# TheaQG/DiffusionModelsCustom

Hardware: NVIDIA B200
Metric: samples_per_s_T1000_ddpm_sampling (higher is better)
Workload: dtype fp16 operands, fp32 accumulate (fp32 state/update)

## Files before the change

### diffusionmodelscustom_b200/csrc/attention_tc8.cuh

```cuda
#pragma once
#include "attention_tc6.cuh"

namespace b2d {

constexpr int AT8_THREADS = 160;
constexpr int AT8_EQ_BYTES = ATC_BLK * ATC_D * 2;
constexpr int AT8_EK_BYTES = (ATC_BN / 2) * ATC_D * 2;
constexpr int AT8_SMEM = 1024 + ATC_TILE_BYTES + ATC_KV_BYTES * 3 * ATC_STAGES + AT8_EQ_BYTES + AT8_EK_BYTES + 256;

constexpr float AT8_OFF_SFU = 7.0f, AT8_OFF_POLY = 22.0f;

__device__ __forceinline__ uint32_t ex2_pair_poly_off(float xa, float xb) {
    uint32_t h, xr, nf, f, p, r;
    asm("cvt.rn.relu.f16x2.f32 %0, %1, %2;" : "=r"(h) : "f"(xb), "f"(xa));
    asm("add.rn.f16x2 %0, %1, %2;" : "=r"(xr) : "r"(h), "r"(0x66006600u));
    asm("sub.rn.f16x2 %0, %1, %2;" : "=r"(nf) : "r"(xr), "r"(0x66006600u));
    asm("sub.rn.f16x2 %0, %1, %2;" : "=r"(f) : "r"(h), "r"(nf));
    asm("fma.rn.f16x2 %0, %1, %2, %3;" : "=r"(p) : "r"(0x2B0D2B0Du), "r"(f), "r"(0x33C333C3u));
    asm("fma.rn.f16x2 %0, %1, %2, %3;" : "=r"(p) : "r"(p), "r"(f), "r"(0x398C398Cu));
    asm("fma.rn.f16x2 %0, %1, %2, %3;" : "=r"(p) : "r"(p), "r"(f), "r"(0x3C003C00u));
    const uint32_t e = xr * 1024u - 0x01980000u;
    asm("mul.rn.f16x2 %0, %1, %2;" : "=r"(r) : "r"(p), "r"(e));
    return r;
}

template <int POLY>
__global__ void __launch_bounds__(AT8_THREADS, AT6_CTAS_PER_SM)
    attn_tc8_kernel(const __grid_constant__ CUtensorMap tm, const __grid_constant__ CUtensorMap tmkv, f16* __restrict__ o, int L,
                    int C, float scale_log2e) {
    pdl_launch_dependents();
    extern __shared__ uint8_t at8_raw[];
    uint8_t* smem = reinterpret_cast<uint8_t*>((reinterpret_cast<uintptr_t>(at8_raw) + 1023) & ~uintptr_t(1023));
    uint8_t* sQ = smem;
    uint8_t* sK = sQ + ATC_TILE_BYTES;
    uint8_t* sV = sK + ATC_STAGES * ATC_KV_BYTES;
    uint8_t* sEq = sV + ATC_STAGES * 2 * ATC_KV_BYTES;
    uint8_t* sEk = sEq + AT8_EQ_BYTES;
    uint64_t* bars = reinterpret_cast<uint64_t*>(sEk + AT8_EK_BYTES);
    constexpr int KV_FULL = 0, S_FULL = 4 , P_EMPTY = 6, Q_FULL = 7, NBARS = 8;
    uint32_t* tmem_slot = reinterpret_cast<uint32_t*>(bars + NBARS);
    const uint32_t bar0 = smem_u32(bars);

    const int warp = threadIdx.x >> 5, lane = threadIdx.x & 31;
    const int head = blockIdx.y, b = blockIdx.z;
    const int q0 = blockIdx.x * ATC_BLK;
    const int nb = L / ATC_BN;
    const int row_base = b * L;
    constexpr int IW = 4, NT = AT8_THREADS;

    if (warp == IW) {
        if (lane == 0) {
            tma_prefetch_desc(&tm);
            tma_prefetch_desc(&tmkv);
            for (int i = 0; i < NBARS; ++i) mbar_init(&bars[i], 1);
            fence_mbar_init();
        }
        __syncwarp();
        tmem_alloc(tmem_slot, AT3_TMEM_COLS);
        tmem_relinquish();
    }
    for (int i = threadIdx.x; i < ATC_STAGES * ATC_BN * 2; i += NT) {
        const int st = i / (ATC_BN * 2), r = i % (ATC_BN * 2);
        *reinterpret_cast<uint4*>(sV + st * 2 * ATC_KV_BYTES + ATC_KV_BYTES + r * 16) = make_uint4(0x00003C00u, 0u, 0u, 0u);
    }
    for (int i = threadIdx.x; i < AT8_EQ_BYTES / 16; i += NT) *reinterpret_cast<uint4*>(sEq + i * 16) = make_uint4(0u, 0x00003C00u, 0u, 0u);
    for (int i = threadIdx.x; i < AT8_EK_BYTES / 16; i += NT) {
        const int pair = (i >> 1) >> 1;
        const uint32_t half_off = ((pair & 7) < POLY) ? 0x4980u  : 0x4300u ;
        *reinterpret_cast<uint4*>(sEk + i * 16) = make_uint4(0x38003800u, half_off, 0u, 0u);
    }
    fence_proxy_async();
    tc_fence_before();
    __syncthreads();
    tc_fence_after();
    const uint32_t tmem = *tmem_slot;
    pdl_wait();

    if (warp == IW) {
        constexpr uint32_t idesc_s = umma_idesc_f16_ex(128, ATC_BN / 2, 0);
        constexpr uint32_t idesc_o = umma_idesc_f16_ex(128, 2 * ATC_D, 1);
        const uint64_t dq = umma_desc(smem_u32(sQ), 0, 256, 6);
        const uint64_t dk0 = umma_desc(smem_u32(sK), 0, 256, 6);
        const uint64_t dv0 = umma_desc(smem_u32(sV), ATC_KV_BYTES, 256, 6);
        const uint64_t deq = umma_desc(smem_u32(sEq), 0, 256, 6);
        const uint64_t dek = umma_desc(smem_u32(sEk), 0, 256, 6);
        constexpr uint64_t K_HALF = (ATC_BN / 2) * ATC_D * 2 / 16;
        auto load_kv = [&](int t) {
            const int st = t & (ATC_STAGES - 1);
            mbar_arrive_expect_tx(&bars[KV_FULL + st], 2 * ATC_KV_BYTES);
            tma_load_2d(sK + st * ATC_KV_BYTES, &tmkv, &bars[KV_FULL + st], C + head * ATC_D, row_base + t * ATC_BN);
            tma_load_2d(sV + st * 2 * ATC_KV_BYTES, &tmkv, &bars[KV_FULL + st], 2 * C + head * ATC_D, row_base + t * ATC_BN);
        };
        auto issue_s_half = [&](int t, int ch) {
            const int ks = t & (ATC_STAGES - 1);
            mbar_wait_a(bar0 + 8 * (KV_FULL + ks), (t >> 2) & 1);
            tc_fence_after();
            const uint32_t d = tmem + ch * (ATC_BN / 2);
            umma_f16(d, dq, dk0 + (uint64_t)(ks * (ATC_KV_BYTES / 16)) + (uint64_t)ch * K_HALF, idesc_s, 0);
            umma_f16(d, deq, dek, idesc_s, 1);
            umma_commit_a(bar0 + 8 * (S_FULL + ch));
        };
        if (elect_one()) {
            mbar_arrive_expect_tx(&bars[Q_FULL], ATC_TILE_BYTES);
            tma_load_2d(sQ, &tm, &bars[Q_FULL], head * ATC_D, row_base + q0);
            const int pre = nb < ATC_STAGES ? nb : ATC_STAGES;
            for (int t = 0; t < pre; ++t) load_kv(t);
        }
// ... 103 lines not shown
                    }
                    if (__any_sync(0xffffffffu, move)) {
                        if (!waited_p) {
                            mbar_wait_a(bar0 + 8 * P_EMPTY, (j & 1) ^ 1);
                            tc_fence_after();
                            waited_p = true;
                        }
                        const float fac = move ? ex2_approx(m_ref - m_new) : 1.0f;
                        if (j > 0) rescale_o(fac);
                        if (ch == 1) rescale_p_first_half(fac);
                        if (j + 1 < nb) mbar_wait_a(bar0 + 8 * (S_FULL + 0), (j + 1) & 1);
                        if (ch == 0) mbar_wait_a(bar0 + 8 * (S_FULL + 1), j & 1);
                        else if (j + 1 < nb) mbar_wait_a(bar0 + 8 * (S_FULL + 1), (j + 1) & 1);
                        if (move) {
                            const f16 hi = __float2half_rn(m_new);
                            const f16 lo = __float2half_rn(m_new - __half2float(hi));
                            const uint32_t w = (uint32_t)__half_as_ushort(__hneg(hi)) | ((uint32_t)__half_as_ushort(__hneg(lo)) << 16);
                            eq_row[0] = w;
                            eq_row[4] = w;
                            m_eq = m_new;
                        }
                        fence_proxy_async();
                    }
                    const float shift = m_new - (m_ref - d0);
#pragma unroll
                    for (int i = 0; i < 32; ++i) v[i] = __float_as_uint(__uint_as_float(v[i]) - shift);
                    m_ref = m_new;
                }
                uint32_t pk[16];
#pragma unroll
                for (int idx = 0; idx < 16 + AT_PIPE; ++idx) {
                    if (idx < 16) {
                        const float s0 = __uint_as_float(v[2 * idx]), s1 = __uint_as_float(v[2 * idx + 1]);
                        if ((idx & 7) < POLY) {
                            pk[idx] = ex2_pair_poly_off(s0, s1);
                        } else {
                            v[2 * idx] = __float_as_uint(ex2_ordered(s0));
                            v[2 * idx + 1] = __float_as_uint(ex2_ordered(s1));
                        }
                    }
                    if (idx >= AT_PIPE) {
                        const int i = idx - AT_PIPE;
                        if ((i & 7) >= POLY) pk[i] = pack_h2_ordered(__uint_as_float(v[2 * i]), __uint_as_float(v[2 * i + 1]));
                    }
                }
                if (!waited_p) {
                    mbar_wait_a(bar0 + 8 * P_EMPTY, (j & 1) ^ 1);
                    tc_fence_after();
                    waited_p = true;
                }
                tmem_st16(tl + AT3_P_COL + ch * 16, pk);
            }
            tmem_st_wait();
            tc_fence_before();
            named_bar_arrive(3, NT);
        }
        mbar_wait_a(bar0 + 8 * P_EMPTY, (nb - 1) & 1);
        tc_fence_after();
        uint32_t ov[32];
        tmem_ld32(tl + AT3_O_COL, ov);
        tmem_ld_wait();
        const float inv = 1.0f / __uint_as_float(ov[16]);
        f16* op = o + ((size_t)(row_base + q0 + row)) * C + head * ATC_D;
        uint4 o0, o1;
        o0.x = pack_h2(__uint_as_float(ov[0]) * inv, __uint_as_float(ov[1]) * inv);
        o0.y = pack_h2(__uint_as_float(ov[2]) * inv, __uint_as_float(ov[3]) * inv);
        o0.z = pack_h2(__uint_as_float(ov[4]) * inv, __uint_as_float(ov[5]) * inv);
        o0.w = pack_h2(__uint_as_float(ov[6]) * inv, __uint_as_float(ov[7]) * inv);
        o1.x = pack_h2(__uint_as_float(ov[8]) * inv, __uint_as_float(ov[9]) * inv);
        o1.y = pack_h2(__uint_as_float(ov[10]) * inv, __uint_as_float(ov[11]) * inv);
        o1.z = pack_h2(__uint_as_float(ov[12]) * inv, __uint_as_float(ov[13]) * inv);
        o1.w = pack_h2(__uint_as_float(ov[14]) * inv, __uint_as_float(ov[15]) * inv);
        reinterpret_cast<uint4*>(op)[0] = o0;
        reinterpret_cast<uint4*>(op)[1] = o1;
    }
    tc_fence_before();
    __syncthreads();
    if (warp == IW) {
        tc_fence_after();
        tmem_dealloc(tmem, AT3_TMEM_COLS);
    }
}

inline int attn_tc8_poly() {
    static const int v = [] {
        const char* e = getenv("B2D_ATTN_POLY");
        const int p = e ? atoi(e) : 4;
        return p < 0 ? 0 : (p > 5 ? 5 : p);
    }();
    return v;
}

template <int POLY>
inline int attn_tc8_attr() {
    B2D_CUDA(cudaFuncSetAttribute(attn_tc8_kernel<POLY>, cudaFuncAttributeMaxDynamicSharedMemorySize, AT8_SMEM));
    B2D_CUDA(cudaFuncSetAttribute(attn_tc8_kernel<POLY>, cudaFuncAttributePreferredSharedMemoryCarveout, cudaSharedmemCarveoutMaxShared));
    return 0;
}
inline int attn_tc8_init_attrs() {
    B2D_TRY(attn_tc8_attr<0>());
    B2D_TRY(attn_tc8_attr<2>());
    B2D_TRY(attn_tc8_attr<3>());
    B2D_TRY(attn_tc8_attr<4>());
    B2D_TRY(attn_tc8_attr<5>());
    return 0;
}

inline int attn_tc8_launch(const AttnTcMaps& m, f16* o, int B, int L, int C, int heads, cudaStream_t st) {
    const float scale_log2e = 1.4426950408889634f / sqrtf((float)ATC_D);
    const dim3 grid(L / ATC_BLK, heads, B), block(AT8_THREADS);
    switch (attn_tc8_poly()) {
        case 0: case 1: B2D_CUDA(launch_k(attn_tc8_kernel<0>, grid, block, AT8_SMEM, st, m.q, m.kv, o, L, C, scale_log2e)); break;
        case 2: B2D_CUDA(launch_k(attn_tc8_kernel<2>, grid, block, AT8_SMEM, st, m.q, m.kv, o, L, C, scale_log2e)); break;
        case 3: B2D_CUDA(launch_k(attn_tc8_kernel<3>, grid, block, AT8_SMEM, st, m.q, m.kv, o, L, C, scale_log2e)); break;
        case 4: B2D_CUDA(launch_k(attn_tc8_kernel<4>, grid, block, AT8_SMEM, st, m.q, m.kv, o, L, C, scale_log2e)); break;
        default: B2D_CUDA(launch_k(attn_tc8_kernel<5>, grid, block, AT8_SMEM, st, m.q, m.kv, o, L, C, scale_log2e)); break;
    }
    return 0;
}

}
```

### diffusionmodelscustom_b200/csrc/b200ddpm.cu

```cuda
#include "../../include/b200ddpm.h"

#include <chrono>
#include <cmath>
#include <cstring>
#include <functional>
#include <map>
#include <memory>
#include <vector>

#include "attention.cuh"
#include "attention_tc.cuh"
#include "attention_tc2.cuh"
#include "attention_tc3.cuh"
#include "attention_tc3d32.cuh"
#include "attention_tc6.cuh"
#include "attention_tc8.cuh"
#include "attn_block.cuh"
#include "common.cuh"
#include "conv.cuh"
#include "conv_persist.cuh"
#include "elementwise.cuh"
#include "evalops.cuh"
#include "gemm_stream.cuh"
#include "norm_fused.cuh"
#include "tail_tc.cuh"

namespace b2d {
thread_local Status g_status;
int g_pdl_enabled = getenv("B2D_NO_PDL") ? 0 : 1;

static inline cudaStream_t as_stream(void* s) { return reinterpret_cast<cudaStream_t>(s); }

struct HostTensor {
    std::vector<float> v;
    std::vector<int64_t> shape;
    size_t numel() const { return v.size(); }
};

static inline uint16_t f2h(float f) {
    const float c = f > 65504.0f ? 65504.0f : (f < -65504.0f ? -65504.0f : f);
    const __half h = __float2half_rn(c);
    uint16_t u;
    memcpy(&u, &h, 2);
    return u;
}

typedef std::function<int(cudaStream_t)> OpFn;
struct Op {
    std::string name;
    std::string klass;
    double flops = 0;
    double bytes = 0;
    OpFn fn;
    bool side = false;
    bool join = false;
    int operator()(cudaStream_t st) const { return fn(st); }
};
struct OpList {
    std::vector<Op> v;
    Op pending;
    void meta(const std::string& name, const std::string& klass, double flops, double bytes) {
        pending.name = name; pending.klass = klass; pending.flops = flops; pending.bytes = bytes;
    }
    void push_back(OpFn f) {
        pending.fn = std::move(f);
        v.push_back(pending);
        pending = Op();
    }
};

struct EnsembleRes;
void ensemble_release(EnsembleRes* r);
struct Handle {
    b2d_config cfg{};
    int num_sms = 148;
    std::vector<void*> allocs;
    std::vector<void*> prog_allocs;
    bool in_prog = false;
    std::map<std::string, HostTensor> sd;
    std::map<std::string, void*> dev;
    bool weights_loaded = false;

    int T = 0;
    float *d_betas = nullptr, *d_alphas = nullptr, *d_alpha_hat = nullptr;

    int prog_B = 0;
    std::vector<Op> step_ops;
    size_t stats_floats = 0;
    float* d_stats = nullptr;
    const float* cur_x = nullptr;
    float* cur_eps = nullptr;
    float* d_eps = nullptr;
    int *d_t = nullptr, *d_step = nullptr, *d_y = nullptr;
    bool has_y = false, has_cond_set = false;
    float* d_cond_stack = nullptr;
    float* d_cond_pre = nullptr;
    float* d_temb = nullptr;
    int n_temb = 0;
    float* d_noise_stage = nullptr;
// ... 363 lines not shown
            auto gp = std::make_shared<GemmStreamPlan>();
            gp->p = p;
            if (gemm_stream_plan_build(*gp, h->num_sms) != 0) { err = -1; return; }
            ops.pending.klass = "gemm_stream";
            ops.push_back([gp](cudaStream_t st) { return gemm_stream_launch(*gp, st); });
        } else {
            if (conv_plan_build(*pl, h->num_sms) != 0) { err = -1; return; }
            static const bool no_gn_epi = getenv("B2D_NO_GN_EPILOGUE") != nullptr;
            const int hw_out = pl->p.Ho * pl->p.Wo;
            const bool gn_whole = pl->p.TN == 1;
            const bool gn_quarter = pl->p.TN > 1 && hw_out % 32 == 0;
            if (want_gn && !no_gn_epi && pl->p.splits == 1 && (gn_whole || gn_quarter) && !convt) {
                const int sub = gn_whole ? 1 : 4;
                const int mtiles = (int)pl->grid.x * sub, ntiles = (int)pl->grid.y;
                float* part = nullptr;
                if (h->alloc(&part, (size_t)mtiles * ntiles * 2) != 0) { err = -2; return; }
                pl->p.gn_partial = part;
                pl->p.gn_sub = sub;
                last_gn_partial = part;
                last_gn_tps = gn_whole ? pl->p.tiles_w * pl->p.tiles_h : hw_out / 32;
                last_gn_ntiles = ntiles;
                last_gn_mtiles = mtiles;
            }
            if (pl->ws_floats) {
                if (h->alloc(&pl->p.ws, pl->ws_floats) != 0) { err = -2; return; }
            }
            if (conv_tcp_eligible(*pl, h->num_sms)) {
                const int sms = h->num_sms;
                ops.pending.klass = "conv_tc";
                ops.push_back([pl, sms](cudaStream_t st) { return conv_launch_tcp(*pl, sms, st); });
            } else {
                ops.push_back([pl](cudaStream_t st) { return conv_launch_tc(*pl, st); });
            }
        }
    }

    f16 *s_xn = nullptr, *s_qkv = nullptr, *s_ao = nullptr, *s_h1 = nullptr, *s_mid = nullptr;

    void attention(const f16* x, int hw, int C, const std::string& role, f16* out, int final_act) {
        const int rows = B * hw * hw, L = hw * hw, heads = h->cfg.n_heads;
        const float* g = W<float>(role + ".ln.g");
        const float* b = W<float>(role + ".ln.b");
        f16 *xn = s_xn, *qkv = s_qkv, *ao = s_ao;
        const int Bc = B;
        static const bool no_ln_fold = getenv("B2D_NO_LN_FOLD") != nullptr;
        const bool fold = !no_ln_fold && !h->cfg.debug_simt_conv && !getenv("B2D_NO_STREAM_GEMM") && C <= 128 && rows >= GS_MIN_ROWS;
        static const bool no_attn_block = getenv("B2D_NO_ATTN_BLOCK") != nullptr;
        const bool fused_block = !no_attn_block && !h->cfg.debug_simt_conv && attn_block_supported(L, C, heads);
        bool fused_out = false;
        if (fused_block) {
            auto pl = std::make_shared<AttnBlockPlan>();
            if (attn_block_plan_build(*pl, x, W<f16>(role + ".qkvln.w"), W<float>(role + ".qkvln.c1"), W<float>(role + ".qkvln.b"), ao,
                                      rows, C, L, heads) != 0) { err = -1; return; }
            static const bool no_out_fuse = getenv("B2D_NO_ATTN_OUT_FUSE") != nullptr;
            static const int out_fuse_maxc = getenv("B2D_ATTN_OUT_FUSE_MAXC") ? atoi(getenv("B2D_ATTN_OUT_FUSE_MAXC")) : 128;
            static const bool want_gather = getenv("B2D_ATTN_GATHER") != nullptr;
            const bool gather = !no_out_fuse && want_gather && attn_block_gather_supported(C, heads);
            fused_out = gather || (!no_out_fuse && attn_block_out_supported(C, heads) && C <= out_fuse_maxc);
            double fl = 6.0 * rows * C * C + 4.0 * (double)L * L * C * B, by = 4.0 * rows * C + 6.0 * C * C;
            if (fused_out) {
                float* ws = nullptr;
                if (!gather && h->alloc(&ws, attn_block_ws_floats(rows, C, heads)) != 0) { err = -2; return; }
                if (attn_block_plan_fuse_out(*pl, W<f16>(role + ".out.w"), W<float>(role + ".out.b"), x,
                                             h->cfg.attn_ff ? s_mid : out, ws, h->cfg.attn_ff ? 0 : final_act, gather ? 2 : 1) != 0) { err = -1; return; }
                fl += 2.0 * rows * C * C;
                by += 4.0 * rows * C + 2.0 * C * C;
            }
            ops.meta(role + ".attn", "attn_block", fl, by);
            ops.push_back([=](cudaStream_t st) { return attn_block_launch(*pl, st); });
        } else if (fold) {
            next_ln_c1 = W<float>(role + ".qkvln.c1");
            conv(x, hw, hw, C, qkv, 3 * C, 1, 1, 0, false, role + ".qkvln", nullptr, nullptr, 0, 0);
        } else {
            ops.meta(role + ".ln", "layernorm", 0, 4.0 * rows * C);
            ops.push_back([=](cudaStream_t st) { return layernorm_launch(x, g, b, xn, rows, C, st); });
            conv(xn, hw, hw, C, qkv, 3 * C, 1, 1, 0, false, role + ".qkv", nullptr, nullptr, 0, 0);
        }
        static const bool no_tc_attn = getenv("B2D_NO_TC_ATTN") != nullptr;
        if (fused_block) {
        } else if (attn_tc_supported(L, C, heads) && !no_tc_attn) {
            auto tmq = std::make_shared<AttnTcMaps>();
            if (attn_tc_make_map(tmq.get(), qkv, B, L, C) != 0) { err = -1; return; }
            ops.meta(role + ".sdpa", "attn_tc", 4.0 * (double)L * L * C * B, 8.0 * rows * C);
            static const int attn_v = getenv("B2D_ATTN_V") ? atoi(getenv("B2D_ATTN_V")) : 8;
            const int sms = h->num_sms;
            if (attn_v == 2 && attn_tc2_supported(L, C, heads))
                ops.push_back([=](cudaStream_t st) { return attn_tc2_launch(*tmq, ao, Bc, L, C, heads, sms, st); });
            else if (attn_v == 1)
                ops.push_back([=](cudaStream_t st) { return attn_tc_launch(*tmq, ao, Bc, L, C, heads, st); });
            else if (attn_v == 4) {
                auto tm4 = std::make_shared<AttnTcMaps>();
                if (attn_tc4_make_map(tm4.get(), qkv, B, L, C) != 0) { err = -1; return; }
                ops.push_back([=](cudaStream_t st) { return attn_tc4_launch(*tm4, ao, Bc, L, C, heads, st); });
            } else if (attn_v == 6)
                ops.push_back([=](cudaStream_t st) { return attn_tc6_launch<0>(*tmq, ao, Bc, L, C, heads, st); });
            else if (attn_v == 7)
                ops.push_back([=](cudaStream_t st) { return attn_tc6_launch<1>(*tmq, ao, Bc, L, C, heads, st); });
            else if (attn_v == 8)
                ops.push_back([=](cudaStream_t st) { return attn_tc8_launch(*tmq, ao, Bc, L, C, heads, st); });
            else
                ops.push_back([=](cudaStream_t st) { return attn_tc3_launch(*tmq, ao, Bc, L, C, heads, st); });
        } else if (attn_tc5_supported(L, C, heads) && !no_tc_attn) {
            auto tm5 = std::make_shared<AttnTcMaps>();
            if (attn_tc5_make_map(tm5.get(), qkv, B, L, C) != 0) { err = -1; return; }
            ops.meta(role + ".sdpa", "attn_tc32", 4.0 * (double)L * L * C * B, 8.0 * rows * C);
            ops.push_back([=](cudaStream_t st) { return attn_tc5_launch(*tm5, ao, Bc, L, C, heads, st); });
        } else {
            ops.meta(role + ".sdpa", "flash_attn", 4.0 * (double)L * L * C * B, 8.0 * rows * C);
            ops.push_back([=](cudaStream_t st) { return flash_attn_launch(qkv, ao, Bc, L, C, heads, st); });
        }
        if (!h->cfg.attn_ff) {
            if (!fused_out) conv(ao, hw, hw, C, out, C, 1, 1, 0, false, role + ".out", x, nullptr, 0, final_act);
        } else {
            f16* mid = s_mid;
            f16* h1 = s_h1;
            if (!fused_out) conv(ao, hw, hw, C, mid, C, 1, 1, 0, false, role + ".out", x, nullptr, 0, 0);
            const float* g2 = W<float>(role + ".ffln.g");
            const float* b2 = W<float>(role + ".ffln.b");
            if (fold) {
                next_ln_c1 = W<float>(role + ".ff1ln.c1");
                conv(mid, hw, hw, C, h1, C, 1, 1, 0, false, role + ".ff1ln", nullptr, nullptr, 0, 2);
            } else {
                ops.meta(role + ".ffln", "layernorm", 0, 4.0 * rows * C);
                ops.push_back([=](cudaStream_t st) { return layernorm_launch(mid, g2, b2, xn, rows, C, st); });
                conv(xn, hw, hw, C, h1, C, 1, 1, 0, false, role + ".ff1", nullptr, nullptr, 0, 2);
            }
            conv(h1, hw, hw, C, out, C, 1, 1, 0, false, role + ".ff2", mid, nullptr, 0, final_act);
        }
    }

    float* stats_slice(int C) {
        float* p = h->d_stats + h->stats_floats;
        h->stats_floats += (size_t)B * C * 2;
        return p;
    }
    void plane_stats(const f16* x, int hw, int C, float* st) {
        const int HW = hw * hw, Bc = B;
        const int ppc = 256;
        const int nslab = (HW + ppc - 1) / ppc, ngrp = C / 64;
        float* partial = nullptr;
        unsigned int* counters = nullptr;
        if (h->alloc(&partial, (size_t)B * ngrp * nslab * 128) != 0 || h->alloc(&counters, (size_t)B * ngrp) != 0) {
            err = -2;
            return;
        }
        if (cudaMemset(counters, 0, (size_t)B * ngrp * sizeof(unsigned int)) != cudaSuccess) err = -2;
        ops.meta("in_stats", "plane_stats", 0, 2.0 * B * HW * C);
        ops.push_back([=](cudaStream_t s) {
            dim3 grid(nslab, ngrp, Bc);
            B2D_CUDA(launch_k(plane_stats_kernel, dim3(grid), dim3(256), 0, s, x, partial, counters, st, HW, C, ppc));
            B2D_CUDA(cudaGetLastError());
            return 0;
        });
    }
    bool instnorm_fused(const f16* x, const f16* skip, const float* vec, int vec_stride, f16* y, int hw, int C) {
        static const bool off = getenv("B2D_NO_FUSED_NORM") != nullptr;
        const int HW = hw * hw;
        if (off || norm_fused_cluster(HW) == 0) return false;
        NormParams np{};
        np.x = x; np.y = y; np.add = skip; np.vec = vec; np.vec_stride = vec_stride; np.C = C; np.rows = HW;
        np.slab_stride = (long long)HW * C;
        const int Bc = B, groups = C / 64;
        ops.meta("in_fused", "norm_fused", 0, 2.0 * B * HW * C * (skip ? 3 : 2));
        ops.push_back([=](cudaStream_t s) { return norm_fused_launch<0>(np, Bc, groups, s); });
        return true;
    }
    void instnorm_apply(const f16* x, const float* st, const f16* skip, const float* vec, int vec_stride, f16* y, int hw,
                        int C) {
        const int HW = hw * hw;
        const size_t total8 = (size_t)B * HW * C / 8;
        ops.meta("in_apply", "instnorm_apply", 0, 2.0 * B * HW * C * (skip ? 3 : 2));
        ops.push_back([=](cudaStream_t s) {
            int blocks = (int)std::min<size_t>((total8 + 255) / 256, (size_t)148 * 16);
            B2D_CUDA(launch_k(instnorm_apply_kernel, dim3(blocks), dim3(256), 0, s, x, st, skip, vec, vec_stride, y, HW, C, total8));
            B2D_CUDA(cudaGetLastError());
            return 0;
        });
    }
};

}
#include "family_d.cuh"
// ... 299 lines not shown
            if (e != cudaSuccess)
                return fail(-2, "step op #" + std::to_string(idx) + " failed: " + cudaGetErrorString(e));
        }
        ++idx;
    }
    return 0;
}

static bool temb_pipelined(const Handle* h) {
    static const bool no_pipe = getenv("B2D_NO_TEMB_PIPE") != nullptr;
    return !no_pipe && h->temb_free_op > 0;
}
static int join_temb_side(Handle* h, cudaStream_t st) {
    if (temb_pipelined(h)) B2D_CUDA(cudaStreamWaitEvent(st, h->ev_side_join, 0));
    return 0;
}

static int ddim_prepare(Handle* h) {
    const int T = h->T, S = (int)h->ddim_tau.size();
    B2D_CHECK(S >= 1 && h->ddim_tau[0] <= T - 1, "DDIM timesteps exceed T-1 of the current schedule");
    B2D_CHECK((int)h->h_alpha_hat.size() == T, "internal: host alpha_hat out of date");
    if (!h->ddim_dirty && h->ddim_cap >= T + 1) return 0;
    B2D_CUDA(cudaDeviceSynchronize());
    if (h->ddim_cap < T + 1) {
        h->drop_ddim_graphs();
        h->release(h->d_ddim_tau);
        h->release(h->d_ddim_coef);
        h->d_ddim_tau = nullptr;
        h->d_ddim_coef = nullptr;
        h->ddim_cap = 0;
        B2D_TRY(h->alloc(&h->d_ddim_tau, T + 1));
        B2D_TRY(h->alloc(&h->d_ddim_coef, T + 1));
        h->ddim_cap = T + 1;
    }
    std::vector<int> tau(h->ddim_tau);
    tau.resize(S + 2, 0);
    std::vector<float4> coef(S);
    for (int k = 0; k < S; ++k)
        coef[k] = ddim_coefficients(h->h_alpha_hat[tau[k]], k + 1 < S ? h->h_alpha_hat[tau[k + 1]] : 1.0f, h->ddim_eta);
    B2D_CUDA(cudaMemcpy(h->d_ddim_tau, tau.data(), tau.size() * sizeof(int), cudaMemcpyHostToDevice));
    B2D_CUDA(cudaMemcpy(h->d_ddim_coef, coef.data(), coef.size() * sizeof(float4), cudaMemcpyHostToDevice));
    h->ddim_dirty = false;
    return 0;
}

}

using namespace b2d;

extern "C" {

const char* b2d_last_error(void) { return g_status.msg.c_str(); }
int b2d_abi_version(void) { return B2D_ABI_VERSION; }

int b2d_create(const b2d_config* cfg, b2d_handle** out) {
    B2D_CHECK(cfg && out, "null argument");
    B2D_CHECK(cfg->family == B2D_FAMILY_R || cfg->family == B2D_FAMILY_D, "unknown family");
    B2D_CHECK(is_pow2(cfg->img_size) && cfg->img_size >= 32 && cfg->img_size <= 128, "img_size must be 32, 64 or 128");
    B2D_CHECK(cfg->max_batch >= 1, "max_batch must be positive");
    B2D_CHECK(cfg->c_hr >= 1 && cfg->c_out >= 1, "channel counts must be positive");
    int dev = 0, ndev = 0;
    cudaError_t e = cudaGetDeviceCount(&ndev);
    if (e != cudaSuccess || ndev == 0)
        return fail(-2, "no CUDA device: this library has no CPU fallback (" + std::string(cudaGetErrorString(e)) + ")");
    B2D_CUDA(cudaGetDevice(&dev));
    cudaDeviceProp prop;
    B2D_CUDA(cudaGetDeviceProperties(&prop, dev));
    B2D_CHECK(prop.major == 10, "b200ddpm kernels are compiled for sm_100a only");
    auto* h = new b2d_handle();
    h->cfg = *cfg;
    if (h->cfg.n_heads <= 0) h->cfg.n_heads = 4;
    h->num_sms = prop.multiProcessorCount;
    int rc = 0;
    do {
        if ((rc = conv_tc_init_attrs())) break;
        if ((rc = conv_tcp_init_attrs())) break;
        if ((rc = flash_attn_init_attrs())) break;
        if ((rc = attn_tc_init_attrs())) break;
        if ((rc = attn_tc2_init_attrs())) break;
        if ((rc = attn_tc3_init_attrs())) break;
        if ((rc = attn_tc5_init_attrs())) break;
        if ((rc = attn_tc6_init_attrs())) break;
        if ((rc = attn_tc8_init_attrs())) break;
        if ((rc = tail_tc_init_attrs())) break;
        if ((rc = gemm_stream_init_attrs())) break;
        if ((rc = attn_block_init_attrs())) break;
        if ((rc = norm_fused_init_attrs())) break;
        if ((rc = init_uniform_carveout())) break;
        const int B = cfg->max_batch, H = cfg->img_size;
        const size_t n = (size_t)B * cfg->c_hr * H * H, plane = (size_t)H * H;
        if ((rc = init_batch_buffers(h))) break;
        if ((rc = h->alloc(&h->d_x_work, n))) break;
        if ((rc = h->alloc(&h->d_job, 1))) break;
        if (cfg->family == B2D_FAMILY_R) {
            if (cfg->has_lsm && (rc = h->alloc(&h->d_lsm_stage, (size_t)B * plane))) break;
            if (cfg->has_topo && (rc = h->alloc(&h->d_topo_stage, (size_t)B * plane))) break;
        }
        h->cond_stage_elems = (size_t)B * std::max(cfg->cond_channels, 1) * plane;
        if ((rc = h->alloc(&h->d_cond_stage, h->cond_stage_elems))) break;
        if (cudaMallocHost(reinterpret_cast<void**>(&h->h_y_pinned), (size_t)B * sizeof(int)) != cudaSuccess) {
            rc = fail(-2, "pinned label staging allocation failed");
            break;
        }
    } while (0);
    if (rc) {
        delete h;
        return rc;
    }
    *out = h;
    return 0;
}

void b2d_destroy(b2d_handle* h) { delete h; }

int b2d_load_weights(b2d_handle* h, const b2d_tensor* tensors, int32_t n) {
    B2D_CHECK(h && tensors && n > 0, "null argument");
    B2D_CHECK(!h->weights_loaded, "weights already loaded on this handle (create a new handle to reload)");
    h->sd.clear();
    for (int i = 0; i < n; ++i) {
        const b2d_tensor& t = tensors[i];
        B2D_CHECK(t.name && t.data && t.ndim >= 0 && t.ndim <= 4, "malformed tensor entry");
        HostTensor ht;
        size_t numel = 1;
        for (int d = 0; d < t.ndim; ++d) {
            ht.shape.push_back(t.shape[d]);
            numel *= (size_t)t.shape[d];
        }
        ht.v.assign(t.data, t.data + numel);
        h->sd[t.name] = std::move(ht);
    }
    int rc = (h->cfg.family == B2D_FAMILY_R) ? pack_family_r(h) : pack_family_d(h);
    h->sd.clear();
    if (rc) return rc;
    h->weights_loaded = true;
    return 0;
}

int b2d_set_schedule(b2d_handle* h, const float* betas, const float* alphas, const float* alpha_hat, int32_t T) {
    B2D_CHECK(h && betas && alphas && alpha_hat && T >= 2, "bad schedule");
    B2D_CUDA(cudaDeviceSynchronize());
    if (T != h->T) {
        h->drop_graphs();
        h->release(h->d_betas);
        h->release(h->d_alphas);
        h->release(h->d_alpha_hat);
        h->d_betas = h->d_alphas = h->d_alpha_hat = nullptr;
        h->T = 0;
        B2D_TRY(h->alloc(&h->d_betas, T));
        B2D_TRY(h->alloc(&h->d_alphas, T));
        B2D_TRY(h->alloc(&h->d_alpha_hat, T));
        h->T = T;
    }
    B2D_CUDA(cudaMemcpy(h->d_betas, betas, T * 4, cudaMemcpyHostToDevice));
    B2D_CUDA(cudaMemcpy(h->d_alphas, alphas, T * 4, cudaMemcpyHostToDevice));
    B2D_CUDA(cudaMemcpy(h->d_alpha_hat, alpha_hat, T * 4, cudaMemcpyHostToDevice));
    h->h_alpha_hat.assign(alpha_hat, alpha_hat + T);
    h->ddim_dirty = true;
    return 0;
}

int b2d_set_timesteps(b2d_handle* h, const int32_t* timesteps_host, int32_t n, float eta) {
    B2D_CHECK(h, "null handle");
    if (n == 0) {
        B2D_CHECK(timesteps_host == nullptr, "n == 0 restores the DDPM loop and takes no timesteps");
        h->ddim = false;
        return 0;
// ... 359 lines not shown
    return 0;
}

int b2d_debug_read(b2d_handle* h, const char* name, float* out_host, int64_t max_elems, int32_t* C_out, int32_t* hw_out) {
    B2D_CHECK(h && name && out_host, "null argument");
    auto it = h->taps.find(name);
    if (it == h->taps.end()) return fail(-3, std::string("no such tap: ") + name);
    const size_t n = (size_t)h->prog_B * it->second.hw * it->second.hw * it->second.C;
    B2D_CHECK((int64_t)n <= max_elems, "output buffer too small");
    std::vector<uint16_t> tmp(n);
    B2D_CUDA(cudaDeviceSynchronize());
    B2D_CUDA(cudaMemcpy(tmp.data(), it->second.p, n * 2, cudaMemcpyDeviceToHost));
    for (size_t i = 0; i < n; ++i) {
        __half hv;
        memcpy(&hv, &tmp[i], 2);
        out_host[i] = __half2float(hv);
    }
    if (C_out) *C_out = it->second.C;
    if (hw_out) *hw_out = it->second.hw;
    return 0;
}

int b2d_op_conv2d(const void* in, const void* w, const float* bias, const void* residual, const float* post_add,
                  int32_t post_stride, void* out, int32_t B, int32_t Hi, int32_t Wi, int32_t Cin, int32_t Cout, int32_t R,
                  int32_t S, int32_t stride, int32_t pad, int32_t convt, int32_t act, int32_t impl, void* stream) {
    B2D_CHECK(in && w && out, "null argument");
    B2D_CHECK(R == S, "square filters only");
    ConvPlan pl;
    ConvParams& p = pl.p;
    memset(&p, 0, sizeof(p));
    p.B = B; p.Hi = Hi; p.Wi = Wi; p.Cin = Cin; p.R = R; p.S = S; p.stride = stride; p.pad = pad; p.convt = convt;
    if (convt) {
        p.Ho = Hi; p.Wo = Wi; p.Cout = 4 * Cout; p.CoutT = Cout;
    } else {
        p.Ho = (Hi + 2 * pad - R) / stride + 1;
        p.Wo = (Wi + 2 * pad - S) / stride + 1;
        p.Cout = Cout; p.CoutT = Cout;
    }
    p.in = (const f16*)in; p.w = (const f16*)w; p.bias = bias; p.residual = (const f16*)residual;
    p.post_add = post_add; p.post_stride = post_stride; p.act = act; p.out = (f16*)out;
    if (impl == 1) return conv_launch_simt(p, as_stream(stream));
    int dev = 0, sms = 148;
    cudaGetDevice(&dev);
    cudaDeviceGetAttribute(&sms, cudaDevAttrMultiProcessorCount, dev);
    if (impl == 2 || (impl == 0 && gemm_stream_supported(p) && getenv("B2D_NO_STREAM_GEMM") == nullptr)) {
        B2D_CHECK(gemm_stream_supported(p, impl == 2 ? 0 : GS_MIN_ROWS), "shape not eligible for the streaming GEMM");
        B2D_TRY(gemm_stream_init_attrs());
        GemmStreamPlan gp;
        gp.p = p;
        B2D_TRY(gemm_stream_plan_build(gp, sms));
        return gemm_stream_launch(gp, as_stream(stream));
    }
    B2D_TRY(conv_tc_init_attrs());
    B2D_TRY(conv_plan_build(pl, sms, impl != 4 && impl != 5));
    if (impl == 5) impl = 3;
    if (impl == 3 || (impl == 0 && conv_tcp_eligible(pl, sms))) {
        B2D_CHECK(pl.p.splits == 1, "shape not eligible for the persistent convolution (split-K plan)");
        B2D_TRY(conv_tcp_init_attrs());
        return conv_launch_tcp(pl, sms, as_stream(stream));
    }
    float* ws = nullptr;
    if (pl.ws_floats) {
        B2D_CUDA(cudaMalloc(&ws, pl.ws_floats * sizeof(float)));
        pl.p.ws = ws;
    }
    int rc = conv_launch_tc(pl, as_stream(stream));
    if (ws) {
        cudaStreamSynchronize(as_stream(stream));
        cudaFree(ws);
    }
    return rc;
}

int b2d_op_layernorm(const void* x, const float* gamma, const float* beta, void* y, int32_t rows, int32_t C, void* stream) {
    return layernorm_launch((const f16*)x, gamma, beta, (f16*)y, rows, C, as_stream(stream));
}

int b2d_op_attention(const void* qkv, void* o, int32_t B, int32_t L, int32_t C, int32_t heads, void* stream) {
    B2D_TRY(flash_attn_init_attrs());
    if (attn_tc_supported(L, C, heads) && getenv("B2D_NO_TC_ATTN") == nullptr) {
        B2D_TRY(attn_tc_init_attrs());
        AttnTcMaps tm;
        B2D_TRY(attn_tc_make_map(&tm, (const f16*)qkv, B, L, C));
        const int attn_v = getenv("B2D_ATTN_V") ? atoi(getenv("B2D_ATTN_V")) : 8;
        if (attn_v == 3) {
            B2D_TRY(attn_tc3_init_attrs());
            return attn_tc3_launch(tm, (f16*)o, B, L, C, heads, as_stream(stream));
        }
        if (attn_v == 8) {
            B2D_TRY(attn_tc8_init_attrs());
            return attn_tc8_launch(tm, (f16*)o, B, L, C, heads, as_stream(stream));
        }
        if (attn_v == 6 || attn_v == 7) {
            B2D_TRY(attn_tc6_init_attrs());
            return attn_v == 6 ? attn_tc6_launch<0>(tm, (f16*)o, B, L, C, heads, as_stream(stream))
                               : attn_tc6_launch<1>(tm, (f16*)o, B, L, C, heads, as_stream(stream));
        }
        if (attn_v == 4) {
            B2D_TRY(attn_tc3_init_attrs());
            B2D_TRY(attn_tc4_make_map(&tm, (const f16*)qkv, B, L, C));
            return attn_tc4_launch(tm, (f16*)o, B, L, C, heads, as_stream(stream));
        }
        if (attn_v == 2 && attn_tc2_supported(L, C, heads)) {
            B2D_TRY(attn_tc2_init_attrs());
            int dev = 0, sms = 148;
            cudaGetDevice(&dev);
            cudaDeviceGetAttribute(&sms, cudaDevAttrMultiProcessorCount, dev);
            return attn_tc2_launch(tm, (f16*)o, B, L, C, heads, sms, as_stream(stream));
        }
        return attn_tc_launch(tm, (f16*)o, B, L, C, heads, as_stream(stream));
    }
    if (attn_tc5_supported(L, C, heads) && getenv("B2D_NO_TC_ATTN") == nullptr) {
        B2D_TRY(attn_tc5_init_attrs());
        AttnTcMaps tm5;
        B2D_TRY(attn_tc5_make_map(&tm5, (const f16*)qkv, B, L, C));
        return attn_tc5_launch(tm5, (f16*)o, B, L, C, heads, as_stream(stream));
    }
    return flash_attn_launch((const f16*)qkv, (f16*)o, B, L, C, heads, as_stream(stream));
}

int b2d_op_attn_block(const void* x, const void* w_folded, const float* c1, const float* bias, void* o, int32_t B, int32_t L,
                      int32_t C, int32_t heads, void* stream) {
    B2D_CHECK(attn_block_supported(L, C, heads), "shape not eligible for the fused low-resolution attention");
    B2D_TRY(attn_block_init_attrs());
    AttnBlockPlan pl;
    B2D_TRY(attn_block_plan_build(pl, (const f16*)x, (const f16*)w_folded, c1, bias, (f16*)o, B * L, C, L, heads));
    return attn_block_launch(pl, as_stream(stream));
}

int b2d_op_attn_block_out(const void* x, const void* w_folded, const float* c1, const float* bias, const void* wo,
                          const float* out_bias, void* y, int32_t B, int32_t L, int32_t C, int32_t heads, int32_t final_act,
                          void* stream) {
    B2D_CHECK(attn_block_supported(L, C, heads) && attn_block_out_supported(C, heads), "shape not eligible for the fused attention block");
    B2D_TRY(attn_block_init_attrs());
    AttnBlockPlan pl;
    B2D_TRY(attn_block_plan_build(pl, (const f16*)x, (const f16*)w_folded, c1, bias, nullptr, B * L, C, L, heads));
    float* ws = nullptr;
    B2D_CUDA(cudaMalloc(&ws, attn_block_ws_floats(B * L, C, heads) * sizeof(float)));
    const bool gather = getenv("B2D_ATTN_GATHER") != nullptr && attn_block_gather_supported(C, heads);
    int rc = attn_block_plan_fuse_out(pl, (const f16*)wo, out_bias, (const f16*)x, (f16*)y, ws, final_act, gather ? 2 : 1);
    if (rc == 0) rc = attn_block_launch(pl, as_stream(stream));
    cudaStreamSynchronize(as_stream(stream));
    cudaFree(ws);
    return rc;
}

int b2d_op_instnorm(const void* x, const void* skip, const float* vec, int32_t vec_stride, void* y, float* stats_ws,
                    int32_t B, int32_t HW, int32_t C, void* stream) {
    cudaStream_t st = as_stream(stream);
    (void)stats_ws;
    B2D_CHECK(C % 64 == 0, "C must be a multiple of 64");
    const int nslab = (HW + 255) / 256, ngrp = C / 64;
    float* ws = nullptr;
    const size_t n_stats = (size_t)B * C * 2, n_part = (size_t)B * ngrp * nslab * 128, n_cnt = (size_t)B * ngrp;
    B2D_CUDA(cudaMalloc(&ws, (n_stats + n_part + n_cnt) * 4));
    float* stats = ws;
    float* partial = ws + n_stats;
    unsigned int* counters = reinterpret_cast<unsigned int*>(ws + n_stats + n_part);
    cudaMemsetAsync(counters, 0, n_cnt * 4, st);
    dim3 grid(nslab, ngrp, B);
    B2D_CUDA(launch_k(plane_stats_kernel, dim3(grid), dim3(256), 0, st, (const f16*)x, partial, counters, stats, HW, C, 256));
    const size_t total8 = (size_t)B * HW * C / 8;
    const int blocks = (int)std::min<size_t>((total8 + 255) / 256, (size_t)148 * 16);
    B2D_CUDA(launch_k(instnorm_apply_kernel, dim3(blocks), dim3(256), 0, st, (const f16*)x, stats, (const f16*)skip, vec, vec_stride, (f16*)y, HW, C,
                                                  total8));
    cudaError_t e = cudaGetLastError();
    cudaStreamSynchronize(st);
    cudaFree(ws);
    B2D_CUDA(e);
    return 0;
}

int b2d_op_final_layer(const void* x, const float* w, const float* bias, float* out, int32_t B, int32_t H, int32_t W,
                       int32_t use_mma_sync, void* stream) {
// ... 172 lines not shown
```

Baseline: 26.23.

## Add speculative-exponential attention kernel that checks overflow after computing P

Adds a new attention kernel variant (v9), now the default. It computes the exponentials first using the current running max, then tracks the packed fp16 maxima with u16x2 max ops to detect overflow. It only falls back to the max-update and rescale slow path when an overflow or a pending max shift is detected. The aim is to take the row-max reduction off the common path of softmax, at the cost of recomputing the exponentials when the speculation fails.

```diff
diff --git a/diffusionmodelscustom_b200/csrc/attention_tc8.cuh b/diffusionmodelscustom_b200/csrc/attention_tc8.cuh
--- a/diffusionmodelscustom_b200/csrc/attention_tc8.cuh
+++ b/diffusionmodelscustom_b200/csrc/attention_tc8.cuh
@@ -10,9 +10,13 @@
 
 constexpr float AT8_OFF_SFU = 7.0f, AT8_OFF_POLY = 22.0f;
 
-__device__ __forceinline__ uint32_t ex2_pair_poly_off(float xa, float xb) {
-    uint32_t h, xr, nf, f, p, r;
+__device__ __forceinline__ uint32_t relu_pack_h2(float xa, float xb) {
+    uint32_t h;
     asm("cvt.rn.relu.f16x2.f32 %0, %1, %2;" : "=r"(h) : "f"(xb), "f"(xa));
+    return h;
+}
+__device__ __forceinline__ uint32_t ex2_h2_poly_off(uint32_t h) {
+    uint32_t xr, nf, f, p, r;
     asm("add.rn.f16x2 %0, %1, %2;" : "=r"(xr) : "r"(h), "r"(0x66006600u));
     asm("sub.rn.f16x2 %0, %1, %2;" : "=r"(nf) : "r"(xr), "r"(0x66006600u));
     asm("sub.rn.f16x2 %0, %1, %2;" : "=r"(f) : "r"(h), "r"(nf));
@@ -23,6 +27,7 @@
     asm("mul.rn.f16x2 %0, %1, %2;" : "=r"(r) : "r"(p), "r"(e));
     return r;
 }
+__device__ __forceinline__ uint32_t ex2_pair_poly_off(float xa, float xb) { return ex2_h2_poly_off(relu_pack_h2(xa, xb)); }
 
 template <int POLY>
 __global__ void __launch_bounds__(AT8_THREADS, AT6_CTAS_PER_SM)
@@ -292,12 +297,13 @@
     }
 }
 
+inline int attn_poly_from_env(int dflt) {
+    const char* e = getenv("B2D_ATTN_POLY");
+    const int p = e ? atoi(e) : dflt;
+    return p < 0 ? 0 : (p > 5 ? 5 : p);
+}
 inline int attn_tc8_poly() {
-    static const int v = [] {
-        const char* e = getenv("B2D_ATTN_POLY");
-        const int p = e ? atoi(e) : 4;
-        return p < 0 ? 0 : (p > 5 ? 5 : p);
-    }();
+    static const int v = attn_poly_from_env(4);
     return v;
 }
 
diff --git a/diffusionmodelscustom_b200/csrc/attention_tc9.cuh b/diffusionmodelscustom_b200/csrc/attention_tc9.cuh
--- /dev/null
+++ b/diffusionmodelscustom_b200/csrc/attention_tc9.cuh
@@ -0,0 +1,347 @@
+#pragma once
+#include "attention_tc8.cuh"
+
+namespace b2d {
+
+__device__ __forceinline__ uint32_t max_u16x2(uint32_t a, uint32_t b) {
+    uint32_t r;
+    asm("max.u16x2 %0, %1, %2;" : "=r"(r) : "r"(a), "r"(b));
+    return r;
+}
+
+template <int POLY>
+__global__ void __launch_bounds__(AT8_THREADS, AT6_CTAS_PER_SM)
+    attn_tc9_kernel(const __grid_constant__ CUtensorMap tm, const __grid_constant__ CUtensorMap tmkv, f16* __restrict__ o, int L,
+                    int C, float scale_log2e) {
+    pdl_launch_dependents();
+    extern __shared__ uint8_t at9_raw[];
+    uint8_t* smem = reinterpret_cast<uint8_t*>((reinterpret_cast<uintptr_t>(at9_raw) + 1023) & ~uintptr_t(1023));
+    uint8_t* sQ = smem;
+    uint8_t* sK = sQ + ATC_TILE_BYTES;
+    uint8_t* sV = sK + ATC_STAGES * ATC_KV_BYTES;
+    uint8_t* sEq = sV + ATC_STAGES * 2 * ATC_KV_BYTES;
+    uint8_t* sEk = sEq + AT8_EQ_BYTES;
+    uint64_t* bars = reinterpret_cast<uint64_t*>(sEk + AT8_EK_BYTES);
+    constexpr int KV_FULL = 0, S_FULL = 4 , P_EMPTY = 6, Q_FULL = 7, NBARS = 8;
+    uint32_t* tmem_slot = reinterpret_cast<uint32_t*>(bars + NBARS);
+    const uint32_t bar0 = smem_u32(bars);
+
+    const int warp = threadIdx.x >> 5, lane = threadIdx.x & 31;
+    const int head = blockIdx.y, b = blockIdx.z;
+    const int q0 = blockIdx.x * ATC_BLK;
+    const int nb = L / ATC_BN;
+    const int row_base = b * L;
+    constexpr int IW = 4, NT = AT8_THREADS;
+
+    if (warp == IW) {
+        if (lane == 0) {
+            tma_prefetch_desc(&tm);
+            tma_prefetch_desc(&tmkv);
+            for (int i = 0; i < NBARS; ++i) mbar_init(&bars[i], 1);
+            fence_mbar_init();
+        }
+        __syncwarp();
+        tmem_alloc(tmem_slot, AT3_TMEM_COLS);
+        tmem_relinquish();
+    }
+    for (int i = threadIdx.x; i < ATC_STAGES * ATC_BN * 2; i += NT) {
+        const int st = i / (ATC_BN * 2), r = i % (ATC_BN * 2);
+        *reinterpret_cast<uint4*>(sV + st * 2 * ATC_KV_BYTES + ATC_KV_BYTES + r * 16) = make_uint4(0x00003C00u, 0u, 0u, 0u);
+    }
+    for (int i = threadIdx.x; i < AT8_EQ_BYTES / 16; i += NT) *reinterpret_cast<uint4*>(sEq + i * 16) = make_uint4(0u, 0x00003C00u, 0u, 0u);
+    for (int i = threadIdx.x; i < AT8_EK_BYTES / 16; i += NT) {
+        const int pair = (i >> 1) >> 1;
+        const uint32_t half_off = ((pair & 7) < POLY) ? 0x4980u  : 0x4300u ;
+        *reinterpret_cast<uint4*>(sEk + i * 16) = make_uint4(0x38003800u, half_off, 0u, 0u);
+    }
+    fence_proxy_async();
+    tc_fence_before();
+    __syncthreads();
+    tc_fence_after();
+    const uint32_t tmem = *tmem_slot;
+    pdl_wait();
+
+    if (warp == IW) {
+        constexpr uint32_t idesc_s = umma_idesc_f16_ex(128, ATC_BN / 2, 0);
+        constexpr uint32_t idesc_o = umma_idesc_f16_ex(128, 2 * ATC_D, 1);
+        const uint64_t dq = umma_desc(smem_u32(sQ), 0, 256, 6);
+        const uint64_t dk0 = umma_desc(smem_u32(sK), 0, 256, 6);
+        const uint64_t dv0 = umma_desc(smem_u32(sV), ATC_KV_BYTES, 256, 6);
+        const uint64_t deq = umma_desc(smem_u32(sEq), 0, 256, 6);
+        const uint64_t dek = umma_desc(smem_u32(sEk), 0, 256, 6);
+        constexpr uint64_t K_HALF = (ATC_BN / 2) * ATC_D * 2 / 16;
+        auto load_kv = [&](int t) {
+            const int st = t & (ATC_STAGES - 1);
+            mbar_arrive_expect_tx(&bars[KV_FULL + st], 2 * ATC_KV_BYTES);
+            tma_load_2d(sK + st * ATC_KV_BYTES, &tmkv, &bars[KV_FULL + st], C + head * ATC_D, row_base + t * ATC_BN);
+            tma_load_2d(sV + st * 2 * ATC_KV_BYTES, &tmkv, &bars[KV_FULL + st], 2 * C + head * ATC_D, row_base + t * ATC_BN);
+        };
+        auto issue_s_half = [&](int t, int ch) {
+            const int ks = t & (ATC_STAGES - 1);
+            mbar_wait_a(bar0 + 8 * (KV_FULL + ks), (t >> 2) & 1);
+            tc_fence_after();
+            const uint32_t d = tmem + ch * (ATC_BN / 2);
+            umma_f16(d, dq, dk0 + (uint64_t)(ks * (ATC_KV_BYTES / 16)) + (uint64_t)ch * K_HALF, idesc_s, 0);
+            umma_f16(d, deq, dek, idesc_s, 1);
+            umma_commit_a(bar0 + 8 * (S_FULL + ch));
+        };
+        if (elect_one()) {
+            mbar_arrive_expect_tx(&bars[Q_FULL], ATC_TILE_BYTES);
+            tma_load_2d(sQ, &tm, &bars[Q_FULL], head * ATC_D, row_base + q0);
+            const int pre = nb < ATC_STAGES ? nb : ATC_STAGES;
+            for (int t = 0; t < pre; ++t) load_kv(t);
+        }
+        __syncwarp();
+        named_bar_sync(4, NT);
+        if (elect_one()) {
+            issue_s_half(0, 0);
+            issue_s_half(0, 1);
+        }
+        __syncwarp();
+        for (int j0 = 0; j0 < nb; j0 += 2) {
+#pragma unroll
+            for (int u = 0; u < 2; ++u) {
+                const int j = j0 + u;
+#pragma unroll
+                for (int ch = 0; ch < 2; ++ch) {
+                    named_bar_sync(1 + ch, NT);
+                    tc_fence_after();
+                    if (j + 1 < nb) {
+                        if (elect_one()) issue_s_half(j + 1, ch);
+                        __syncwarp();
+                    }
+                }
+                named_bar_sync(3, NT);
+                tc_fence_after();
+                if (elect_one()) {
+                    const uint64_t dv = dv0 + (uint64_t)(((j0 & 2) + u) * (2 * ATC_KV_BYTES / 16));
+#pragma unroll
+                    for (int kk = 0; kk < ATC_BN / 16; ++kk)
+                        umma_f16_ts(tmem + AT3_O_COL, tmem + AT3_P_COL + kk * 8, dv + (uint64_t)(kk * (512 / 16)), idesc_o, (j | kk) != 0);
+                    umma_commit_a(bar0 + 8 * P_EMPTY);
+                    if (j >= 1 && j + 3 < nb) load_kv(j + 3);
+                }
+                __syncwarp();
+            }
+        }
+    } else {
+        const uint32_t tl = tmem + ((uint32_t)(warp * 32) << 16);
+        const int row = warp * 32 + lane;
+        {
+            mbar_wait_a(bar0 + 8 * Q_FULL, 0);
+            const f162 sc = __float2half2_rn(scale_log2e);
+            f162* qp = reinterpret_cast<f162*>(sQ + threadIdx.x * 32);
+#pragma unroll
+            for (int i = 0; i < 8; ++i) qp[i] = __hmul2(qp[i], sc);
+            fence_proxy_async();
+            named_bar_arrive(4, NT);
+        }
+        uint32_t* eq_row = reinterpret_cast<uint32_t*>(sEq + row * 32);
+        float m_ref = 0.f;
+        float m_eq = 0.f;
+        float mb[2] = {0.f, 0.f};
+        auto rescale_o = [&](float fac) {
+            uint32_t ov[32];
+            tmem_ld32(tl + AT3_O_COL, ov);
+            tmem_ld_wait();
+            uint32_t o0[16], o1[16];
+#pragma unroll
+            for (int i = 0; i < 16; ++i) {
+                o0[i] = __float_as_uint(__uint_as_float(ov[i]) * fac);
+                o1[i] = __float_as_uint(__uint_as_float(ov[16 + i]) * fac);
+            }
+            tmem_st16(tl + AT3_O_COL, o0);
+            tmem_st16(tl + AT3_O_COL + 16, o1);
+            tmem_st_wait();
+        };
+        auto rescale_p_first_half = [&](float fac) {
+            tmem_st_wait();
+            uint32_t pv[32];
+            tmem_ld32(tl + AT3_P_COL, pv);
+            tmem_ld_wait();
+            uint32_t p0[16];
+#pragma unroll
+            for (int i = 0; i < 16; ++i) {
+                const float2 f = unpack_h2(pv[i]);
+                p0[i] = pack_h2_nosat(f.x * fac, f.y * fac);
+            }
+            tmem_st16(tl + AT3_P_COL, p0);
+        };
+        auto exponentials = [&](const uint32_t (&v)[32], uint32_t (&pk)[16]) -> uint32_t {
+            float y[32];
+            uint32_t hmax = 0u, pmax = 0u;
+#pragma unroll
+            for (int idx = 0; idx < 16 + AT_PIPE; ++idx) {
+                if (idx < 16) {
+                    const float s0 = __uint_as_float(v[2 * idx]), s1 = __uint_as_float(v[2 * idx + 1]);
+                    if ((idx & 7) < POLY) {
+                        const uint32_t h = relu_pack_h2(s0, s1);
+                        hmax = max_u16x2(hmax, h);
+                        pk[idx] = ex2_h2_poly_off(h);
+                    } else {
+                        y[2 * idx] = ex2_ordered(s0);
+                        y[2 * idx + 1] = ex2_ordered(s1);
+                    }
+                }
+                if (idx >= AT_PIPE) {
+                    const int i = idx - AT_PIPE;
+                    if ((i & 7) >= POLY) {
+                        pk[i] = pack_h2_ordered(y[2 * i], y[2 * i + 1]);
+                        pmax = max_u16x2(pmax, pk[i]);
+                    }
+                }
+            }
+            return (hmax + 0x30803080u) | (pmax + 0x08000800u);
+        };
+
+        for (int j0 = 0; j0 < nb; j0 += 2) {
+#pragma unroll
+            for (int u = 0; u < 2; ++u) {
+                const int j = j0 + u;
+                bool waited_p = false;
+#pragma unroll
+                for (int ch = 0; ch < 2; ++ch) {
+                    mbar_wait_a(bar0 + 8 * (S_FULL + ch), u);
+                    tc_fence_after();
+                    uint32_t v[32];
+                    tmem_ld32(tl + ch * 32, v);
+                    tmem_ld_wait();
+                    tc_fence_before();
+                    named_bar_arrive(1 + ch, NT);
+                    const float d0 = m_ref - mb[ch];
+                    mb[ch] = m_eq;
+                    const bool first = (j == 0) && (ch == 0);
+                    auto slow_path = [&]() {
+                        float mx[2] = {-INFINITY, -INFINITY};
+#pragma unroll
+                        for (int i = 0; i < 32; i += 2) {
+                            const int cls = (((i >> 1) & 7) < POLY) ? 1 : 0;
+                            mx[cls] = fmaxf(mx[cls], fmaxf(__uint_as_float(v[i]), __uint_as_float(v[i + 1])));
+                        }
+                        const float cm = fmaxf(mx[0] - AT8_OFF_SFU, mx[1] - AT8_OFF_POLY) - d0;
+                        const bool move = cm > 8.0f || first;
+                        float m_new = m_ref;
+                        if (move) {
+                            const float t = m_ref + cm;
+                            const f16 hi = __float2half_rn(t);
+                            const f16 lo = __float2half_rn(t - __half2float(hi));
+                            m_new = __half2float(hi) + __half2float(lo);
+                        }
+                        if (__any_sync(0xffffffffu, move)) {
+                            if (!waited_p) {
+                                mbar_wait_a(bar0 + 8 * P_EMPTY, u ^ 1);
+                                tc_fence_after();
+                                waited_p = true;
+                            }
+                            const float fac = move ? ex2_approx(m_ref - m_new) : 1.0f;
+                            if (j > 0) rescale_o(fac);
+                            if (ch == 1) rescale_p_first_half(fac);
+                            if (j + 1 < nb) mbar_wait_a(bar0 + 8 * (S_FULL + 0), u ^ 1);
+                            if (ch == 0) mbar_wait_a(bar0 + 8 * (S_FULL + 1), u);
+                            else if (j + 1 < nb) mbar_wait_a(bar0 + 8 * (S_FULL + 1), u ^ 1);
+                            if (move) {
+                                const f16 hi = __float2half_rn(m_new);
+                                const f16 lo = __float2half_rn(m_new - __half2float(hi));
+                                const uint32_t w = (uint32_t)__half_as_ushort(__hneg(hi)) | ((uint32_t)__half_as_ushort(__hneg(lo)) << 16);
+                                eq_row[0] = w;
+                                eq_row[4] = w;
+                                m_eq = m_new;
+                            }
+                            fence_proxy_async();
+                        }
+                        const float shift = m_new - (m_ref - d0);
+#pragma unroll
+                        for (int i = 0; i < 32; ++i) v[i] = __float_as_uint(__uint_as_float(v[i]) - shift);
+                        m_ref = m_new;
+                    };
+                    auto store_p = [&](const uint32_t (&pk)[16]) {
+                        if (!waited_p) {
+                            mbar_wait_a(bar0 + 8 * P_EMPTY, u ^ 1);
+                            tc_fence_after();
+                            waited_p = true;
+                        }
+                        tmem_st16(tl + AT3_P_COL + ch * 16, pk);
+                    };
+                    uint32_t pk[16];
+                    if (first) {
+                        slow_path();
+                        exponentials(v, pk);
+                        store_p(pk);
+                        continue;
+                    }
+                    const uint32_t over = exponentials(v, pk);
+                    if (__any_sync(0xffffffffu, d0 != 0.0f || (over & 0x80008000u) != 0u)) {
+                        slow_path();
+                        uint32_t pk2[16];
+                        exponentials(v, pk2);
+                        store_p(pk2);
+                    } else {
+                        store_p(pk);
+                    }
+                }
+                tmem_st_wait();
+                tc_fence_before();
+                named_bar_arrive(3, NT);
+            }
+        }
+        mbar_wait_a(bar0 + 8 * P_EMPTY, (nb - 1) & 1);
+        tc_fence_after();
+        uint32_t ov[32];
+        tmem_ld32(tl + AT3_O_COL, ov);
+        tmem_ld_wait();
+        const float inv = 1.0f / __uint_as_float(ov[16]);
+        f16* op = o + ((size_t)(row_base + q0 + row)) * C + head * ATC_D;
+        uint4 o0, o1;
+        o0.x = pack_h2(__uint_as_float(ov[0]) * inv, __uint_as_float(ov[1]) * inv);
+        o0.y = pack_h2(__uint_as_float(ov[2]) * inv, __uint_as_float(ov[3]) * inv);
+        o0.z = pack_h2(__uint_as_float(ov[4]) * inv, __uint_as_float(ov[5]) * inv);
+        o0.w = pack_h2(__uint_as_float(ov[6]) * inv, __uint_as_float(ov[7]) * inv);
+        o1.x = pack_h2(__uint_as_float(ov[8]) * inv, __uint_as_float(ov[9]) * inv);
+        o1.y = pack_h2(__uint_as_float(ov[10]) * inv, __uint_as_float(ov[11]) * inv);
+        o1.z = pack_h2(__uint_as_float(ov[12]) * inv, __uint_as_float(ov[13]) * inv);
+        o1.w = pack_h2(__uint_as_float(ov[14]) * inv, __uint_as_float(ov[15]) * inv);
+        reinterpret_cast<uint4*>(op)[0] = o0;
+        reinterpret_cast<uint4*>(op)[1] = o1;
+    }
+    tc_fence_before();
+    __syncthreads();
+    if (warp == IW) {
+        tc_fence_after();
+        tmem_dealloc(tmem, AT3_TMEM_COLS);
+    }
+}
+
+inline int attn_tc9_poly() {
+    static const int v = attn_poly_from_env(4);
+    return v;
+}
+
+template <int POLY>
+inline int attn_tc9_attr() {
+    B2D_CUDA(cudaFuncSetAttribute(attn_tc9_kernel<POLY>, cudaFuncAttributeMaxDynamicSharedMemorySize, AT8_SMEM));
+    B2D_CUDA(cudaFuncSetAttribute(attn_tc9_kernel<POLY>, cudaFuncAttributePreferredSharedMemoryCarveout, cudaSharedmemCarveoutMaxShared));
+    return 0;
+}
+inline int attn_tc9_init_attrs() {
+    B2D_TRY(attn_tc9_attr<0>());
+    B2D_TRY(attn_tc9_attr<2>());
+    B2D_TRY(attn_tc9_attr<3>());
+    B2D_TRY(attn_tc9_attr<4>());
+    B2D_TRY(attn_tc9_attr<5>());
+    return 0;
+}
+
+inline int attn_tc9_launch(const AttnTcMaps& m, f16* o, int B, int L, int C, int heads, cudaStream_t st) {
+    const float scale_log2e = 1.4426950408889634f / sqrtf((float)ATC_D);
+    const dim3 grid(L / ATC_BLK, heads, B), block(AT8_THREADS);
+    switch (attn_tc9_poly()) {
+        case 0: case 1: B2D_CUDA(launch_k(attn_tc9_kernel<0>, grid, block, AT8_SMEM, st, m.q, m.kv, o, L, C, scale_log2e)); break;
+        case 2: B2D_CUDA(launch_k(attn_tc9_kernel<2>, grid, block, AT8_SMEM, st, m.q, m.kv, o, L, C, scale_log2e)); break;
+        case 3: B2D_CUDA(launch_k(attn_tc9_kernel<3>, grid, block, AT8_SMEM, st, m.q, m.kv, o, L, C, scale_log2e)); break;
+        case 4: B2D_CUDA(launch_k(attn_tc9_kernel<4>, grid, block, AT8_SMEM, st, m.q, m.kv, o, L, C, scale_log2e)); break;
+        default: B2D_CUDA(launch_k(attn_tc9_kernel<5>, grid, block, AT8_SMEM, st, m.q, m.kv, o, L, C, scale_log2e)); break;
+    }
+    return 0;
+}
+
+}
diff --git a/diffusionmodelscustom_b200/csrc/b200ddpm.cu b/diffusionmodelscustom_b200/csrc/b200ddpm.cu
--- a/diffusionmodelscustom_b200/csrc/b200ddpm.cu
+++ b/diffusionmodelscustom_b200/csrc/b200ddpm.cu
@@ -15,6 +15,7 @@
 #include "attention_tc3d32.cuh"
 #include "attention_tc6.cuh"
 #include "attention_tc8.cuh"
+#include "attention_tc9.cuh"
 #include "attn_block.cuh"
 #include "common.cuh"
 #include "conv.cuh"
@@ -544,7 +545,7 @@
             auto tmq = std::make_shared<AttnTcMaps>();
             if (attn_tc_make_map(tmq.get(), qkv, B, L, C) != 0) { err = -1; return; }
             ops.meta(role + ".sdpa", "attn_tc", 4.0 * (double)L * L * C * B, 8.0 * rows * C);
-            static const int attn_v = getenv("B2D_ATTN_V") ? atoi(getenv("B2D_ATTN_V")) : 8;
+            static const int attn_v = getenv("B2D_ATTN_V") ? atoi(getenv("B2D_ATTN_V")) : 9;
             const int sms = h->num_sms;
             if (attn_v == 2 && attn_tc2_supported(L, C, heads))
                 ops.push_back([=](cudaStream_t st) { return attn_tc2_launch(*tmq, ao, Bc, L, C, heads, sms, st); });
@@ -560,6 +561,8 @@
                 ops.push_back([=](cudaStream_t st) { return attn_tc6_launch<1>(*tmq, ao, Bc, L, C, heads, st); });
             else if (attn_v == 8)
                 ops.push_back([=](cudaStream_t st) { return attn_tc8_launch(*tmq, ao, Bc, L, C, heads, st); });
+            else if (attn_v == 9)
+                ops.push_back([=](cudaStream_t st) { return attn_tc9_launch(*tmq, ao, Bc, L, C, heads, st); });
             else
                 ops.push_back([=](cudaStream_t st) { return attn_tc3_launch(*tmq, ao, Bc, L, C, heads, st); });
         } else if (attn_tc5_supported(L, C, heads) && !no_tc_attn) {
@@ -1025,6 +1028,7 @@
         if ((rc = attn_tc5_init_attrs())) break;
         if ((rc = attn_tc6_init_attrs())) break;
         if ((rc = attn_tc8_init_attrs())) break;
+        if ((rc = attn_tc9_init_attrs())) break;
         if ((rc = tail_tc_init_attrs())) break;
         if ((rc = gemm_stream_init_attrs())) break;
         if ((rc = attn_block_init_attrs())) break;
@@ -1550,7 +1554,7 @@
         B2D_TRY(attn_tc_init_attrs());
         AttnTcMaps tm;
         B2D_TRY(attn_tc_make_map(&tm, (const f16*)qkv, B, L, C));
-        const int attn_v = getenv("B2D_ATTN_V") ? atoi(getenv("B2D_ATTN_V")) : 8;
+        const int attn_v = getenv("B2D_ATTN_V") ? atoi(getenv("B2D_ATTN_V")) : 9;
         if (attn_v == 3) {
             B2D_TRY(attn_tc3_init_attrs());
             return attn_tc3_launch(tm, (f16*)o, B, L, C, heads, as_stream(stream));
@@ -1558,6 +1562,10 @@
         if (attn_v == 8) {
             B2D_TRY(attn_tc8_init_attrs());
             return attn_tc8_launch(tm, (f16*)o, B, L, C, heads, as_stream(stream));
+        }
+        if (attn_v == 9) {
+            B2D_TRY(attn_tc9_init_attrs());
+            return attn_tc9_launch(tm, (f16*)o, B, L, C, heads, as_stream(stream));
         }
         if (attn_v == 6 || attn_v == 7) {
             B2D_TRY(attn_tc6_init_attrs());
```

Measured after the change: 26.38 (median of 6 runs). About the same (+0.6%).
